# sbelharbi/feature-vs-text-compound-emotion

Hardware: AMD Instinct MI355X
Metric: training clips/sec (32-frame tri-modal clip) (higher is better)
Workload: dtype bf16x3 (split hi/lo bf16 operands, 3 MFMAs per product, fp32 accumulate; <= 2^-15 relative per product)

## Files before the change

feature_vs_text_compound_emotion_amd/csrc/conv_b3.h:

```cpp
#pragma once
#include "conv_common.h"

namespace cer {

typedef __bf16 bf16x8 __attribute__((ext_vector_type(8)));
typedef unsigned int u32x4 __attribute__((ext_vector_type(4)));
typedef __attribute__((address_space(3))) void *lds_ptr_t;

__device__ __forceinline__ bf16x8 as_bf16x8(const u32x4 v) { return __builtin_bit_cast(bf16x8, v); }


typedef float f32x4 __attribute__((ext_vector_type(4)));
__device__ __forceinline__ int swz16(int q) { return (0x78 >> (2 * q)) & 3; }

int conv_b3_patch_launch(int tile, const ConvArgs &a, hipStream_t st);
bool conv_b3_patch_ok(const ConvArgs &a);
bool conv_b3_win_ok(const ConvArgs &a);
int conv_b3_s2d_launch(int tile, const ConvArgs &a, hipStream_t st);
bool conv_b3_s2d_ok(const ConvArgs &a);

}
```

feature_vs_text_compound_emotion_amd/csrc/conv_b3.hip:

```cpp
#include "conv_b3.h"

namespace cer {

template <int BM, int BN, int WP, int WC, int NW = 4, int STAGES = 2>
__global__ __launch_bounds__(NW * 64, NW == 4 ? 2 : 1) void conv_b3_dma16_kernel(ConvArgs p) {
    static_assert(WP * WC == NW && BM % (16 * NW) == 0 && BN % (16 * NW) == 0, "1-KiB pieces are dealt round-robin to the waves");
    constexpr int BKT = 32, ROWB = BKT * 2;
    constexpr int XP = BM / (16 * NW), WQ = BN / (16 * NW);
    constexpr int PX = BM * ROWB, PW = BN * ROWB;
    constexpr int BUF = 2 * PX + 2 * PW;
    constexpr int NDMA = 2 * XP + 2 * WQ;
    static_assert(STAGES == 2 || STAGES == 3, "ring depth");
    constexpr int TP = BM / (16 * WP), TC = BN / (16 * WC);
    constexpr unsigned OOB = 0x80000000u;
    extern __shared__ __attribute__((aligned(16))) uint16_t smem_b3[];
    unsigned char *smem = reinterpret_cast<unsigned char *>(smem_b3);

    const int tid = threadIdx.x, lane = tid & 63;
    const int wave = __builtin_amdgcn_readfirstlane(tid >> 6);
    const int wp = wave % WP, wc = wave / WP;
    const int kg = lane >> 4, l15 = lane & 15;

    const int nwg = p.tiles_m * p.tiles_n;
    int bid = blockIdx.x;
// ... 247 lines not shown
                    const int m = m0 + (wp * TP + b) * 16 + l15;
                    const float v = (m < p.M) ? acc[a][b][r] : 0.f;
                    s1 += v;
                    s2 += v * v;
                });
#pragma unroll
                for (int o = 8; o > 0; o >>= 1) {
                    s1 += __shfl_xor(s1, o);
                    s2 += __shfl_xor(s2, o);
                }
                if (l15 == 0) {
                    const int ci = (wc * TC + a) * 16 + 4 * kg + r;
                    red[(wp * 2 + 0) * BN + ci] = s1;
                    red[(wp * 2 + 1) * BN + ci] = s2;
                }
            });
        });
        __syncthreads();
        if (tid < BN && c0 + tid < p.Cout) {
            float s1 = 0.f, s2 = 0.f;
#pragma unroll
            for (int w = 0; w < WP; ++w) {
                s1 += red[(w * 2 + 0) * BN + tid];
                s2 += red[(w * 2 + 1) * BN + tid];
            }
            p.stats[((size_t)tile_m * 2 + 0) * p.Cout + c0 + tid] = s1;
            p.stats[((size_t)tile_m * 2 + 1) * p.Cout + c0 + tid] = s2;
        }
    }
}

__global__ void split_bf16_kernel(const float4 *__restrict__ x, const float *__restrict__ scale,
                                  const float *__restrict__ shift, ushort4 *__restrict__ hi, ushort4 *__restrict__ lo,
                                  size_t n4, int C4) {
    size_t i = (size_t)blockIdx.x * blockDim.x + threadIdx.x;
    if (i >= n4) return;
    float4 v = x[i];
    if (scale) {
        const int c = (int)(i % C4) * 4;
        const float4 s = *reinterpret_cast<const float4 *>(scale + c), t = *reinterpret_cast<const float4 *>(shift + c);
        v = make_float4(v.x * s.x + t.x, v.y * s.y + t.y, v.z * s.z + t.z, v.w * s.w + t.w);
    }
    ushort4 h, l;
    split_bf16(v.x, h.x, l.x); split_bf16(v.y, h.y, l.y);
    split_bf16(v.z, h.z, l.z); split_bf16(v.w, h.w, l.w);
    hi[i] = h;
    lo[i] = l;
}

template <int BM, int BN, int WP, int WC, int NW = 4, int STAGES = 2>
static int launch_b3_dma16(const ConvArgs &a, hipStream_t st) {
    if ((long long)BN * a.Kpad * 2 >= (1ll << 31))
        return cer_set_error(CER_ERR_UNSUPPORTED, "conv2d (bf16x3, LDS-DMA): weight panel exceeds 31-bit offsets");
    const size_t lds = (size_t)STAGES * (2 * BM + 2 * BN) * 64;
    auto k = conv_b3_dma16_kernel<BM, BN, WP, WC, NW, STAGES>;
    if (lds > 64 * 1024) CER_HIP_CHECK(hipFuncSetAttribute((const void *)k, hipFuncAttributeMaxDynamicSharedMemorySize, (int)lds));
    CER_LAUNCH(k, dim3(a.tiles_m * a.tiles_n, 1, a.split_k), dim3(NW * 64), lds, st, a);
    CER_HIP_CHECK(hipGetLastError());
    return CER_OK;
}

static bool b3_patch_geometry(const cer_conv_desc *d) {
    return d->KH == 3 && d->KW == 3 && d->stride == 1 && d->dil_h == 1 && d->dil_w == 1 && d->pad_t == 1 && d->pad_l == 1 &&
           d->Ho == d->H && d->Wo == d->W && (d->H & 15) == 0 && (d->W & 15) == 0 && (d->Cin & 31) == 0 && d->split_k <= 1;
}

static bool b3_win_geometry(const cer_conv_desc *d) {
    return d->KH == 3 && d->KW == 3 && d->stride == 1 && d->dil_h == 1 && d->dil_w == 1 && d->pad_t == 1 && d->pad_l == 1 &&
           d->Ho == d->H && d->Wo == d->W && d->H >= 2 && d->W >= 2 && d->W <= 86 && (d->Cin & 31) == 0 && d->split_k <= 1;
}

int conv_b3_tile_dims(const cer_conv_desc *d, int &bm, int &bn, int &bk) {
    int tile = d->tile;
    const long long M = (long long)d->N * d->Ho * d->Wo;
    const int Cout = d->Cout;
    if (d->x_s2d) {
        if (tile == 0) tile = Cout > 64 ? 52 : 51;
        else if (tile != 51 && tile != 52) return 0;
    } else if (tile == 51 || tile == 52) {
        return 0;
    }
    if (tile == 0) {
        const long long t128 = (M + 127) / 128 * ((Cout + 127) / 128), t256 = (M + 255) / 256;
        if (b3_patch_geometry(d) && Cout <= 64 && t256 >= 512) tile = 59;
        else if (b3_patch_geometry(d) && Cout >= 128 && t256 * ((Cout + 127) / 128) >= 512) tile = 58;
        else if (b3_win_geometry(d) && t256 >= 64) tile = Cout > 64 ? 56 : 53;
        else if (Cout <= 64) tile = t256 >= 512 ? 48 : 42;
        else if (t128 >= 512) tile = 41;
        else tile = Cout >= 128 ? 44 : 45;
    }
    bk = 32;
    switch (tile) {
        case 41: bm = 128; bn = 128; break;
        case 42: bm = 128; bn = 64; break;
        case 44: bm = 64; bn = 128; break;
        case 45: bm = 64; bn = 64; break;
        case 48: bm = 256; bn = 64; break;
        case 59: bm = 256; bn = 64; break;
        case 58: bm = 256; bn = 128; break;
        case 53: bm = 256; bn = 64; break;
        case 56: bm = 256; bn = 128; break;
        case 51: bm = 256; bn = 64; break;
        case 52: bm = 256; bn = 128; break;
        default: return 0;
    }
    return tile;
}

int conv_b3_launch(int tile, const ConvArgs &a, hipStream_t st) {
    switch (tile) {
        case 41: return launch_b3_dma16<128, 128, 2, 2>(a, st);
        case 42: return launch_b3_dma16<128, 64, 2, 2>(a, st);
        case 44: return launch_b3_dma16<64, 128, 1, 4>(a, st);
        case 45: return launch_b3_dma16<64, 64, 2, 2>(a, st);
        case 48: return launch_b3_dma16<256, 64, 4, 1>(a, st);
        case 53: case 56: case 58: case 59: return conv_b3_patch_launch(tile, a, st);
        case 51: case 52: return conv_b3_s2d_launch(tile, a, st);
        default: return cer_set_error(CER_ERR_INVALID_ARG, "conv2d (bf16x3): unknown tile id");
    }
}

}

using namespace cer;

extern "C" int cer_conv2d_b3_tile(const cer_conv_desc *d) {
    if (!d || d->N <= 0 || d->Ho <= 0 || d->Wo <= 0 || d->Cout <= 0) return 0;
    int bm, bn, bk;
    return conv_b3_tile_dims(d, bm, bn, bk);
}

extern "C" int cer_split_bf16(const float *x, const float *scale, const float *shift, int C, uint16_t *hi, uint16_t *lo,
                              size_t n, void *stream) {
    if (!x || !hi || !lo || n == 0 || (n & 3)) return cer_set_error(CER_ERR_INVALID_ARG, "split_bf16: n must be a positive multiple of 4");
    if ((scale == nullptr) != (shift == nullptr) || (scale && (C <= 0 || (C & 3) || n % C)))
        return cer_set_error(CER_ERR_INVALID_ARG, "split_bf16: the per-channel affine needs scale, shift and C % 4 == 0 dividing n");
    CER_LAUNCH(split_bf16_kernel, dim3(cer_blocks(n / 4, 256)), dim3(256), 0, (hipStream_t)stream, (const float4 *)x, scale,
               shift, (ushort4 *)hi, (ushort4 *)lo, n / 4, scale ? C / 4 : 1);
    CER_HIP_CHECK(hipGetLastError());
    return CER_OK;
}
```

feature_vs_text_compound_emotion_amd/csrc/conv_igemm.hip:

```cpp
#include <hip/hip_runtime.h>
#include <stdint.h>

#include "cer_internal.h"
#include "conv_common.h"

namespace cer {

template <int BM, int BN, int WP, int WC, bool VEC, int VAR, int BKT>
__global__ __launch_bounds__(WP * WC * 64, 3) void conv_igemm_kernel(ConvArgs p) {
    constexpr int NT = WP * WC * 64;
    constexpr int CH = BKT / 4;
    constexpr int RPP = NT / CH;
    constexpr int PIT = BKT + 4;
    constexpr int NG = BKT / 8;
    constexpr bool PRIO = (VAR & 1) != 0, SINGLE = (VAR & 2) != 0, BLKPRIO = (VAR & 4) != 0;
    constexpr bool ABL_NOSTAGE = (VAR & 8) != 0;
    constexpr bool ABL_NOBAR = (VAR & 16) != 0;
    constexpr int NBUF = SINGLE ? 1 : 2;
    constexpr int TP = BM / (32 * WP);
    constexpr int TC = BN / (32 * WC);
    constexpr int XR = BM / RPP;
    constexpr int WR = BN / RPP;
    extern __shared__ __attribute__((aligned(16))) float smem[];
    float *Xs = smem;
// ... 316 lines not shown
        if (t.bn > 64 && d->Cout <= 64) continue;
        const long long blocks = (long long)((M + t.bm - 1) / t.bm) * ((d->Cout + t.bn - 1) / t.bn) * d->split_k;
        const long long slots = 256ll * t.per_cu;
        const long long rounds = (blocks + slots - 1) / slots;
        const float frac = (float)(blocks - (rounds - 1) * slots) / (float)slots;
        const float eff_rounds = (float)(rounds - 1) + (frac < 0.5f ? 0.5f + frac * 0.5f : (frac < 1.f ? 0.75f + frac * 0.25f : 1.f));
        const float time = eff_rounds * (float)(t.bm * t.bn) * (float)t.per_cu / t.rate;
        if (time < best_t) { best_t = time; best = t.id; }
    }
    return best;
}

static void tile_dims(int tile, int &bm, int &bn) {
    switch (tile) {
        case 1: bm = 128; bn = 128; break;
        case 2: bm = 128; bn = 64; break;
        case 4: bm = 64; bn = 128; break;
        default: bm = 64; bn = 64; break;
    }
}

template <int VAR>
static int launch_shape(int shape, const ConvArgs &a, bool vec, hipStream_t st) {
    switch (shape) {
        case 1: return launch_cfg<128, 128, 2, 2, VAR>(a, vec, st);
        case 2: return launch_cfg<128, 64, 2, 2, VAR>(a, vec, st);
        case 4: return launch_cfg<64, 128, 1, 4, VAR>(a, vec, st);
        case 5: return launch_cfg<64, 64, 2, 2, VAR>(a, vec, st);
        default: return cer_set_error(CER_ERR_INVALID_ARG, "conv2d_fwd: unknown tile id");
    }
}

}

using namespace cer;

extern "C" int cer_conv_kpad(int KH, int KW, int Cin) {
    int K = KH * KW * Cin;
    return (K + BK - 1) / BK * BK;
}

static int validate_desc(const cer_conv_desc *d) {
    if (!d) return cer_set_error(CER_ERR_INVALID_ARG, "conv desc is NULL");
    if (d->N <= 0 || d->H <= 0 || d->W <= 0 || d->Cin <= 0 || d->Ho <= 0 || d->Wo <= 0 || d->Cout <= 0 ||
        d->KH <= 0 || d->KW <= 0 || d->stride <= 0 || d->dil_h <= 0 || d->dil_w <= 0 || d->split_k < 1)
        return cer_set_error(CER_ERR_INVALID_ARG, "conv desc: non-positive dimension");
    if ((long long)d->N * d->Ho * d->Wo >= (1ll << 31) || (long long)d->N * d->H * d->W >= (1ll << 31))
        return cer_set_error(CER_ERR_UNSUPPORTED, "conv desc: more than 2^31 pixels");
    if (d->x_nchw && (d->Cin % 32) == 0)
        return cer_set_error(CER_ERR_UNSUPPORTED, "conv desc: NCHW input only on the small-Cin path");
    return CER_OK;
}

namespace cer {
int conv_b3_tile_dims(const cer_conv_desc *d, int &bm, int &bn, int &bk);
int conv_n16_tile_dims(const cer_conv_desc *d, int &bm, int &bn, int &bk);
}

extern "C" int cer_conv2d_stats_tiles(const cer_conv_desc *d, int kernel_family) {
    if (!d || d->N <= 0 || d->Ho <= 0 || d->Wo <= 0) return 0;
    const int M = d->N * d->Ho * d->Wo;
    int bm, bn, bk;
    if (kernel_family == 2) {
        if (!conv_n16_tile_dims(d, bm, bn, bk)) return 0;
    } else if (kernel_family == 1) {
        const int t = conv_b3_tile_dims(d, bm, bn, bk);
        if (!t) return 0;
        if (t == 6) return 2 * ((M + bm - 1) / bm);
    } else {
        tile_dims(pick_tile(d, M), bm, bn);
    }
    return (M + bm - 1) / bm;
}

extern "C" size_t cer_conv2d_workspace_bytes(const cer_conv_desc *d) {
    if (!d || d->split_k <= 1) return 0;
    return (size_t)d->split_k * d->N * d->Ho * d->Wo * d->Cout * sizeof(float);
}

namespace cer {
int conv_b3_launch(int tile, const ConvArgs &a, hipStream_t st);
int conv_n16_launch(int tile, const ConvArgs &a, hipStream_t st);
bool conv_n16_p64_ok(const ConvArgs &a);
}

extern "C" int cer_conv2d_run(const cer_conv_desc *d, const cer_conv_io *io, void *workspace, size_t workspace_bytes,
                              void *stream) {
    int rc = validate_desc(d);
    if (rc) return rc;
    if (!io) return cer_set_error(CER_ERR_INVALID_ARG, "conv2d: io block is NULL");
    if (d->storage != CER_STORE_NONE && d->storage != CER_STORE_BF16 && d->storage != CER_STORE_F16)
        return cer_set_error(CER_ERR_INVALID_ARG, "conv2d: unknown storage type");
    const bool narrow = d->storage != CER_STORE_NONE;
    const bool n16 = narrow && io->x_hi != nullptr;
    const bool b3 = !narrow && io->x_hi != nullptr;
    if (narrow && (io->x_lo || io->w_lo || io->y_lo || io->res_lo || io->y2_hi || io->y2_lo))
        return cer_set_error(CER_ERR_INVALID_ARG, "conv2d (narrow): 16-bit tensors are single planes (every *_lo and y2 pointer must be NULL)");
    if (n16) {
        if (!io->w_hi) return cer_set_error(CER_ERR_INVALID_ARG, "conv2d (narrow): x_hi and w_hi must both be given");
        if (io->in_scale || io->mask || io->aux || d->x_nchw)
            return cer_set_error(CER_ERR_UNSUPPORTED, "conv2d (narrow): no input affine / mask / aux / NCHW input");
    } else if (b3) {
        if (!io->x_lo || !io->w_hi || !io->w_lo)
            return cer_set_error(CER_ERR_INVALID_ARG, "conv2d (bf16x3): x_hi, x_lo, w_hi, w_lo must all be given");
        if (io->in_scale || io->mask || io->aux || d->x_nchw)
            return cer_set_error(CER_ERR_UNSUPPORTED, "conv2d (bf16x3): no input affine / mask / aux / NCHW input");
    } else if (!io->x || !io->w) {
        return cer_set_error(CER_ERR_INVALID_ARG, "conv2d: x and w must be non-NULL");
    }
    if (!io->y && !io->y_hi && !io->y2_hi) return cer_set_error(CER_ERR_INVALID_ARG, "conv2d: no output tensor");
    if ((io->in_scale == nullptr) != (io->in_shift == nullptr))
        return cer_set_error(CER_ERR_INVALID_ARG, "conv2d: in_scale and in_shift go together");
    if (!narrow && ((io->y_hi == nullptr) != (io->y_lo == nullptr) || (io->res_hi == nullptr) != (io->res_lo == nullptr) ||
                    (io->y2_hi == nullptr) != (io->y2_lo == nullptr) || (io->y2_hi && (!io->s2 || !io->t2))))
        return cer_set_error(CER_ERR_INVALID_ARG, "conv2d: split tensors need both planes (and s2/t2 for the second output)");
    if (io->residual && io->res_hi) return cer_set_error(CER_ERR_INVALID_ARG, "conv2d: give the residual as fp32 OR split");
    if (d->act1 == CER_ACT_PRELU && !io->alpha) return cer_set_error(CER_ERR_INVALID_ARG, "conv2d: PReLU needs alpha");
    const bool has_res = io->residual || io->res_hi;
    if (has_res && (d->res_stride <= 0 || d->Hr <= 0 || d->Wr <= 0 || (d->Ho - 1) * d->res_stride >= d->Hr ||
                    (d->Wo - 1) * d->res_stride >= d->Wr))
        return cer_set_error(CER_ERR_INVALID_ARG, "conv2d: residual geometry out of range");
    if (io->stats && d->split_k > 1)
        return cer_set_error(CER_ERR_UNSUPPORTED, "conv2d: batch statistics are not available with split-K");
    if ((io->y_hi || io->y2_hi || io->res_hi) && (d->Cout & 3))
        return cer_set_error(CER_ERR_UNSUPPORTED, "conv2d: split outputs / residual need Cout % 4 == 0");
    ConvArgs a{};
    a.x = io->x; a.w = io->w; a.in_scale = io->in_scale; a.in_shift = io->in_shift; a.bias = io->bias; a.alpha = io->alpha;
    a.res = io->residual; a.mask = io->mask; a.y = io->y; a.aux = io->aux; a.stats = io->stats;
    a.x_hi = io->x_hi; a.x_lo = io->x_lo; a.w_hi = io->w_hi; a.w_lo = io->w_lo;
    a.res_hi = io->res_hi; a.res_lo = io->res_lo; a.y_hi = io->y_hi; a.y_lo = io->y_lo;
    a.s2 = io->s2; a.t2 = io->t2; a.y2_hi = io->y2_hi; a.y2_lo = io->y2_lo;
    a.bias9 = io->bias9;
    a.narrow = d->storage;
    if (io->bias9 && (io->bias || d->stride != 1 || d->Ho != d->H || d->Wo != d->W || d->H < 2 || d->W < 2 || d->split_k > 1))
        return cer_set_error(CER_ERR_INVALID_ARG, "conv2d: bias9 replaces bias and needs a stride-1 same conv on >= 2x2 images without split-K");
    if (d->x_s2d || d->y_s2d) {
        if (!b3 && !n16) return cer_set_error(CER_ERR_UNSUPPORTED, "conv2d: space-to-depth tensors exist in the bf16x3 and narrow modes only");
        if (d->x_s2d && d->x_ld > 0) return cer_set_error(CER_ERR_INVALID_ARG, "conv2d: x_s2d fixes the input pitch (x_ld must be 0)");
        if (d->y_s2d && ((d->Ho | d->Wo) & 1 || io->y || io->y2_hi || has_res || io->mask || io->aux || d->y_ld > 0 || !io->y_hi))
            return cer_set_error(CER_ERR_INVALID_ARG, "conv2d: y_s2d needs even Ho / Wo and a plain 16-bit output (no fp32 / second "
                                                      "output, residual, mask, aux or y_ld)");
    }
    a.x_s2d = d->x_s2d != 0; a.y_s2d = d->y_s2d != 0;
    a.x_ld = d->x_s2d ? 4 * d->Cin : (d->x_ld > 0 ? d->x_ld : d->Cin);
    a.y_ld = d->y_ld > 0 ? d->y_ld : d->Cout;
    if (a.x_ld < d->Cin || a.y_ld < d->Cout || ((d->Cin % 32) == 0 && (a.x_ld & 3) != 0))
        return cer_set_error(CER_ERR_INVALID_ARG, "conv2d: x_ld/y_ld smaller than the channel count or x_ld % 4 != 0");
    if (d->x_nchw && d->x_ld > 0) return cer_set_error(CER_ERR_INVALID_ARG, "conv2d: x_ld is meaningless for NCHW input");
    a.N = d->N; a.H = d->H; a.W = d->W; a.Cin = d->Cin; a.Ho = d->Ho; a.Wo = d->Wo; a.Cout = d->Cout;
    a.KH = d->KH; a.KW = d->KW; a.stride = d->stride; a.dil_h = d->dil_h; a.dil_w = d->dil_w;
    a.pad_t = d->pad_t; a.pad_l = d->pad_l; a.x_nchw = d->x_nchw;
    a.res_stride = d->res_stride; a.Hr = d->Hr; a.Wr = d->Wr; a.act1 = d->act1; a.act2 = d->act2;
    a.slope = d->slope;
    a.Kpad = cer_conv_kpad(d->KH, d->KW, d->Cin);
    a.M = d->N * d->Ho * d->Wo;
    const bool vec = (d->Cin % 32) == 0;
    int tile, bm, bn, bk, esz;
    if (n16) {
        tile = conv_n16_tile_dims(d, bm, bn, bk);
        if (!tile) return cer_set_error(CER_ERR_INVALID_ARG, "conv2d (narrow): unknown tile id (space-to-depth input: 81 / 82 only)");
        if (d->y_s2d && tile != 71 && tile != 72 && tile != 78 && tile != 73 && tile != 76 && tile != 77 && tile != 79)
            return cer_set_error(CER_ERR_UNSUPPORTED, "conv2d (narrow): y_s2d is written by the window / patch kernels only "
                                                      "(cer_conv2d_n16_tile(desc) in {71, 72, 73, 76, 77, 78, 79})");
        if (d->Cin % bk != 0 || (a.x_ld & 7))
            return cer_set_error(CER_ERR_UNSUPPORTED, "conv2d (narrow): Cin must be a multiple of 64 and x_ld of 8");
        esz = 2;
    } else if (b3) {
        tile = conv_b3_tile_dims(d, bm, bn, bk);
        if (!tile) return cer_set_error(CER_ERR_INVALID_ARG, "conv2d (bf16x3): unknown tile id (space-to-depth input: 51 / 52 only)");
        if (d->y_s2d && tile != 53 && tile != 56 && tile != 58 && tile != 59)
            return cer_set_error(CER_ERR_UNSUPPORTED, "conv2d (bf16x3): y_s2d is written by the window / patch kernels only "
                                                      "(cer_conv2d_b3_tile(desc) in {53, 56, 58, 59})");
        if (d->Cin % bk != 0 || (a.x_ld & 7))
            return cer_set_error(CER_ERR_UNSUPPORTED, "conv2d (bf16x3): Cin must be a multiple of the K step and x_ld of 8");
        esz = 2;
    } else {
        tile = pick_tile(d, a.M);
        if (tile != 1 && tile != 2 && tile != 4 && tile != 5) return cer_set_error(CER_ERR_INVALID_ARG, "conv2d: unknown tile id");
        bk = 32;
        tile_dims(tile, bm, bn);
        esz = 4;
    }
    a.cin_steps = (vec || b3 || n16) ? d->Cin / bk : 1;
    a.steps = a.Kpad / bk;
    a.split_k = d->split_k > a.steps ? a.steps : d->split_k;
    a.steps_per_split = (a.steps + a.split_k - 1) / a.split_k;
    a.split_k = (a.steps + a.steps_per_split - 1) / a.steps_per_split;
    a.tiles_m = (a.M + bm - 1) / bm;
    a.tiles_n = (a.Cout + bn - 1) / bn;
    if (vec || b3 || n16) {
        if (d->KH * d->KW > 32) return cer_set_error(CER_ERR_UNSUPPORTED, "conv2d: more than 32 filter taps");
        if (d->Wo > d->W / d->stride + 1 ||
            (long long)d->H * d->W < (long long)(d->Ho - 1) * d->stride * d->W + (long long)(d->Wo - 1) * d->stride)
            return cer_set_error(CER_ERR_UNSUPPORTED, "conv2d: the output grid outruns the input (Ho/Wo too large for H/W and stride)");
        const long long span_px = (long long)bm * d->stride * d->stride + 2ll * d->H * d->W + (long long)d->W * d->stride + 2;
        if (span_px * a.x_ld * esz >= (1ll << 31) || (long long)bn * a.Kpad * esz >= (1ll << 32))
            return cer_set_error(CER_ERR_UNSUPPORTED, "conv2d: tile footprint exceeds 32-bit staging offsets");
    }
    hipStream_t st = (hipStream_t)stream;
    ConvArgs fin = a;
    if (a.split_k > 1) {
        size_t need = (size_t)a.split_k * a.M * a.Cout * sizeof(float);
        if (!workspace || workspace_bytes < need) return cer_set_error(CER_ERR_WORKSPACE, "conv2d: split-K workspace too small");
        a.y = (float *)workspace;
    }
    if (n16) {
        if (tile == 79 && d->tile == 0 && !conv_n16_p64_ok(a)) tile = 71;
        rc = conv_n16_launch(tile, a, st);
    } else if (b3) {
        rc = conv_b3_launch(tile, a, st);
    } else {
        rc = launch_shape<2>(tile, a, vec, st);
    }
    if (rc) return rc;
    if (a.split_k > 1) {
        fin.split_k = a.split_k;
        size_t n = (size_t)a.M * ((a.Cout + 3) / 4);
        CER_LAUNCH(splitk_reduce_kernel, dim3((unsigned)((n + 255) / 256)), dim3(256), 0, st, fin, (const float *)workspace);
        CER_HIP_CHECK(hipGetLastError());
    }
    return CER_OK;
}

extern "C" int cer_conv2d_fwd(const cer_conv_desc *d, const float *x, const float *w, const float *in_scale,
                              const float *in_shift, const float *bias, const float *alpha, const float *residual,
                              const float *mask, float *y, float *aux, float *stats, void *workspace,
                              size_t workspace_bytes, void *stream) {
    if (!x || !w || !y) return cer_set_error(CER_ERR_INVALID_ARG, "conv2d_fwd: x, w, y must be non-NULL");
    cer_conv_io io{};
    io.x = x; io.w = w; io.in_scale = in_scale; io.in_shift = in_shift; io.bias = bias; io.alpha = alpha;
    io.residual = residual; io.mask = mask; io.y = y; io.aux = aux; io.stats = stats;
    return cer_conv2d_run(d, &io, workspace, workspace_bytes, stream);
}
```

feature_vs_text_compound_emotion_amd/ops.py:

```python
import ctypes
import os

import torch

from . import _lib
from ._lib import (ACT_GELU, ACT_LEAKY, ACT_NONE, ACT_PRELU, ACT_RELU, STORE_BF16, STORE_F16, STORE_NONE, ConvDesc,
                   ConvIO, check, current_stream, ptr)

LEAKY_SLOPE = 0.01


def _dev_f32(t, name, contiguous=True, shape=None):
    if t is None:
        return
    if not (t.is_cuda and t.dtype == torch.float32 and (t.is_contiguous() or not contiguous)):
        raise ValueError(f"{name}: expected a contiguous float32 tensor on the GPU, got "
                         f"{t.dtype} {t.device} contiguous={t.is_contiguous()}")
    if shape is not None and tuple(t.shape) != tuple(shape):
        raise ValueError(f"{name}: expected shape {tuple(shape)}, got {tuple(t.shape)}")


def _dev_mask(mask, y):
    _dev_f32(mask, "mask")
    if mask is not None and mask.numel() != y.numel():
# ... 79 lines not shown
            raise ValueError("y_ld needs an explicit out buffer")
        out = _empty((n, ho, wo, cout), x)
    elif out is not None:
        _dev_f32(out, "out", contiguous=(y_ld == 0))
    ws_bytes = lib.cer_conv2d_workspace_bytes(ctypes.byref(d))
    ws = _empty((ws_bytes // 4,), x) if ws_bytes else None
    stats = _empty((lib.cer_conv2d_stats_tiles(ctypes.byref(d), 0), 2, cout), x) if want_stats else None
    if out_n16 is not None:
        if out_split or next_affine is not None:
            raise ValueError("out_n16 excludes the split outputs")
        io = ConvIO()
        io.x, io.w = x.data_ptr(), w_packed.data_ptr()
        for name, t in (("in_scale", in_scale), ("in_shift", in_shift), ("bias", bias), ("alpha", alpha),
                        ("residual", residual), ("mask", mask), ("y", out), ("aux", aux), ("stats", stats)):
            if t is not None:
                setattr(io, name, t.data_ptr())
        d.storage = storage_of(out_n16)
        res = {"y": out, "stats": stats, "n16": torch.empty((n, ho, wo, cout), device=x.device, dtype=out_n16)}
        io.y_hi = res["n16"].data_ptr()
        check(lib.cer_conv2d_run(ctypes.byref(d), ctypes.byref(io), ptr(ws), ws_bytes, current_stream()), "cer_conv2d_run")
        return res
    if not (out_split or next_affine is not None):
        check(lib.cer_conv2d_fwd(ctypes.byref(d), ptr(x), ptr(w_packed), ptr(in_scale), ptr(in_shift), ptr(bias),
                                 ptr(alpha), ptr(residual), ptr(mask), ptr(out), ptr(aux), ptr(stats), ptr(ws), ws_bytes,
                                 current_stream()), "cer_conv2d_fwd")
        return (out, stats) if want_stats else out
    io = ConvIO()
    io.x, io.w = x.data_ptr(), w_packed.data_ptr()
    for name, t in (("in_scale", in_scale), ("in_shift", in_shift), ("bias", bias), ("alpha", alpha),
                    ("residual", residual), ("mask", mask), ("y", out), ("aux", aux), ("stats", stats)):
        if t is not None:
            setattr(io, name, t.data_ptr())
    res = {"y": out, "stats": stats}
    if out_split:
        res["split"] = Split.empty((n, ho, wo, cout), x.device)
        io.y_hi, io.y_lo = res["split"].hi.data_ptr(), res["split"].lo.data_ptr()
    if next_affine is not None:
        s2, t2 = next_affine
        res["next"] = Split.empty((n, ho, wo, cout), x.device)
        io.s2, io.t2 = s2.data_ptr(), t2.data_ptr()
        io.y2_hi, io.y2_lo = res["next"].hi.data_ptr(), res["next"].lo.data_ptr()
    check(lib.cer_conv2d_run(ctypes.byref(d), ctypes.byref(io), ptr(ws), ws_bytes, current_stream()), "cer_conv2d_run")
    return res


class Split:
    __slots__ = ("hi", "lo")

    def __init__(self, hi, lo):
        self.hi, self.lo = hi, lo

    @property
    def shape(self):
        return self.hi.shape

    def float(self):
        return self.hi.float() + self.lo.float()

    def view(self, *shape):
        return Split(self.hi.view(*shape), self.lo.view(*shape))

    @staticmethod
    def empty(shape, device):
        return Split(torch.empty(shape, device=device, dtype=torch.bfloat16),
                     torch.empty(shape, device=device, dtype=torch.bfloat16))


def split_bf16(x, scale=None, shift=None):
    _dev_f32(x, "x")
    _dev_f32(scale, "scale", shape=x.shape[-1:])
    _dev_f32(shift, "shift", shape=x.shape[-1:])
    out = Split.empty(x.shape, x.device)
    c = x.shape[-1] if scale is not None else 0
    check(_lib.load().cer_split_bf16(ptr(x), ptr(scale), ptr(shift), c, ptr(out.hi), ptr(out.lo), x.numel(),
                                     current_stream()), "cer_split_bf16")
    return out


def _dev_bf16(t, name):
    if t is not None and not (t.is_cuda and t.dtype == torch.bfloat16 and t.is_contiguous()):
        raise ValueError(f"{name}: expected a contiguous bfloat16 GPU tensor")


CONV_TRACE = None


def conv2d_b3(x, w, kh, kw, *, stride=1, dil=(1, 1), pad=(0, 0), out_hw=None, bias=None, alpha=None, residual=None,
              res_stride=1, act1=ACT_NONE, act2=ACT_NONE, slope=LEAKY_SLOPE, split_k=1, tile=0, out_f32=False,
              out_split=True, next_affine=None, want_stats=False, bias9=None, x_s2d=False, y_s2d=False):
    lib = _lib.load()
    for t, n in ((x.hi, "x.hi"), (x.lo, "x.lo"), (w.hi, "w.hi"), (w.lo, "w.lo")):
        _dev_bf16(t, n)
    _dev_f32(bias, "bias")
    _dev_f32(alpha, "alpha")
    n, h, wd, cin = x.shape
    if x_s2d:
        if cin % 4:
            raise ValueError("a space-to-depth input has 4 * Cin channels")
        h, wd, cin = 2 * h, 2 * wd, cin // 4
    cout = w.shape[0]
    if w.shape[1] != conv_kpad(kh, kw, cin):
        raise ValueError(f"packed weight has K={w.shape[1]}, expected {conv_kpad(kh, kw, cin)}")
    if out_hw is None:
        ho = (h + 2 * pad[0] - dil[0] * (kh - 1) - 1) // stride + 1
        wo = (wd + 2 * pad[1] - dil[1] * (kw - 1) - 1) // stride + 1
    else:
        ho, wo = out_hw
    d = ConvDesc()
    d.N, d.H, d.W, d.Cin, d.Ho, d.Wo, d.Cout = n, h, wd, cin, ho, wo, cout
    d.KH, d.KW, d.stride, d.dil_h, d.dil_w, d.pad_t, d.pad_l = kh, kw, stride, dil[0], dil[1], pad[0], pad[1]
    d.res_stride, d.Hr, d.Wr = res_stride, 0, 0
    d.act1, d.act2, d.slope, d.split_k, d.tile = act1, act2, slope, split_k, tile
    d.x_s2d, d.y_s2d = int(x_s2d), int(y_s2d)
    io = ConvIO()
    io.x_hi, io.x_lo, io.w_hi, io.w_lo = x.hi.data_ptr(), x.lo.data_ptr(), w.hi.data_ptr(), w.lo.data_ptr()
    io.bias = bias.data_ptr() if bias is not None else None
    io.alpha = alpha.data_ptr() if alpha is not None else None
    if bias9 is not None:
        _dev_f32(bias9, "bias9")
        if tuple(bias9.shape) != (9, cout):
            raise ValueError("bias9 must be [9, Cout]")
        io.bias9 = bias9.data_ptr()
    if residual is not None:
        rshape = residual.shape
        if rshape[0] != n or rshape[3] != cout:
            raise ValueError("residual shape does not match the output")
        d.Hr, d.Wr = rshape[1], rshape[2]
        if isinstance(residual, Split):
            _dev_bf16(residual.hi, "residual.hi")
            io.res_hi, io.res_lo = residual.hi.data_ptr(), residual.lo.data_ptr()
        else:
            _dev_f32(residual, "residual")
            io.residual = residual.data_ptr()
    res = {}
    dev = x.hi.device
    if out_f32:
        res["y"] = torch.empty((n, ho, wo, cout), device=dev, dtype=torch.float32)
        io.y = res["y"].data_ptr()
    if out_split:
        res["split"] = Split.empty((n, ho // 2, wo // 2, 4 * cout) if y_s2d else (n, ho, wo, cout), dev)
        io.y_hi, io.y_lo = res["split"].hi.data_ptr(), res["split"].lo.data_ptr()
    if next_affine is not None:
        s2, t2 = next_affine
        _dev_f32(s2, "s2")
        _dev_f32(t2, "t2")
        res["next"] = Split.empty((n, ho, wo, cout), dev)
        io.s2, io.t2 = s2.data_ptr(), t2.data_ptr()
        io.y2_hi, io.y2_lo = res["next"].hi.data_ptr(), res["next"].lo.data_ptr()
    if want_stats:
        res["stats"] = torch.empty((lib.cer_conv2d_stats_tiles(ctypes.byref(d), 1), 2, cout), device=dev,
                                   dtype=torch.float32)
        io.stats = res["stats"].data_ptr()
    ws_bytes = lib.cer_conv2d_workspace_bytes(ctypes.byref(d))
    ws = torch.empty((ws_bytes // 4,), device=dev, dtype=torch.float32) if ws_bytes else None
    if CONV_TRACE is not None:
        e0, e1 = torch.cuda.Event(enable_timing=True), torch.cuda.Event(enable_timing=True)
        e0.record()
    check(lib.cer_conv2d_run(ctypes.byref(d), ctypes.byref(io), ptr(ws), ws_bytes, current_stream()), "cer_conv2d_run")
    if CONV_TRACE is not None:
        e1.record()
        nout = n * ho * wo * cout
        nbytes = 4.0 * n * h * wd * cin + 4.0 * nout * (int(out_f32) + int(out_split) + int(next_affine is not None)) + \
            4.0 * cout * cin * kh * kw + (4.0 * nout if residual is not None else 0.0)
        CONV_TRACE.append((lib.cer_conv2d_b3_tile(ctypes.byref(d)), 2.0 * n * ho * wo * cout * cin * kh * kw, e0, e1, nbytes))
    return res


def stem_conv(x, w, scale=None, shift=None, alpha=None, out=None, want_stats=False):
    _dev_f32(x, "x")
    _dev_f32(w, "w")
    for t, nme in ((scale, "scale"), (shift, "shift"), (alpha, "alpha")):
        _dev_f32(t, nme)
    n, c, h, wd = x.shape
    if c != 3 or w.shape[0] != 64:
        raise ValueError("stem_conv is the 3 -> 64 input layer")
    lib = _lib.load()
    stats = _empty((lib.cer_stem_conv3x3_stats_rows(n, h), 2, 64), x) if (want_stats or out is None) else None
    res, y, hi, lo, storage = {}, None, None, None, STORE_NONE
    if out == "f32":
        res["y"] = y = torch.empty((n, h, wd, 64), device=x.device, dtype=torch.float32)
    elif out == "split":
        res["split"] = Split.empty((n, h, wd, 64), x.device)
        hi, lo = res["split"].hi, res["split"].lo
    elif out is not None:
        storage = storage_of(out)
        res["n16"] = hi = torch.empty((n, h, wd, 64), device=x.device, dtype=out)
    check(lib.cer_stem_conv3x3(ptr(x), ptr(w), w.shape[1], ptr(scale), ptr(shift), ptr(alpha), ptr(y), ptr(hi), ptr(lo), storage,
                               ptr(stats), n, h, wd, current_stream()), "cer_stem_conv3x3")
    if out is None:
        return stats
    if want_stats:
        res["stats"] = stats
    return res


def _tile_desc(n, h, w, cin, cout, kh, kw, stride, pad, x_s2d):
    d = ConvDesc()
    d.N, d.H, d.W, d.Cin, d.Cout = n, h, w, cin, cout
    d.Ho, d.Wo = (h + 2 * pad[0] - kh) // stride + 1, (w + 2 * pad[1] - kw) // stride + 1
    d.KH, d.KW, d.stride, d.dil_h, d.dil_w, d.pad_t, d.pad_l = kh, kw, stride, 1, 1, pad[0], pad[1]
    d.split_k, d.x_s2d = 1, int(x_s2d)
    return d


def conv2d_b3_tile(n, h, w, cin, cout, kh, kw, stride, pad, x_s2d=False):
    return _lib.load().cer_conv2d_b3_tile(ctypes.byref(_tile_desc(n, h, w, cin, cout, kh, kw, stride, pad, x_s2d)))


def conv2d_n16_tile(n, h, w, cin, cout, kh, kw, stride, pad, x_s2d=False):
    return _lib.load().cer_conv2d_n16_tile(ctypes.byref(_tile_desc(n, h, w, cin, cout, kh, kw, stride, pad, x_s2d)))


S2D_PRODUCER_TILES = (53, 56, 58, 59)
S2D_PRODUCER_TILES_N16 = (71, 72, 73, 76, 77, 78, 79)


def s2d_k_order(cin, device, chunk=32):
    order = (ctypes.c_int32 * (9 * cin))()
    check(_lib.load().cer_conv_s2d_k_order(cin, chunk, order), "cer_conv_s2d_k_order")
    return torch.tensor(list(order), dtype=torch.long, device=device)


def pack_s2d_weight(w, cin, chunk=None):
    if isinstance(w, Split):
        idx = s2d_k_order(cin, w.hi.device, chunk or 32)
        return Split(w.hi.index_select(1, idx).contiguous(), w.lo.index_select(1, idx).contiguous())
    return w.index_select(1, s2d_k_order(cin, w.device, chunk or 64)).contiguous()


def space_to_depth(x):
    if isinstance(x, Split):
        return Split(space_to_depth(x.hi), space_to_depth(x.lo))
    return torch.cat([x[:, 1::2, 1::2], x[:, 1::2, 0::2], x[:, 0::2, 1::2], x[:, 0::2, 0::2]], dim=3).contiguous()


def storage_of(dtype):
    if dtype == torch.bfloat16:
        return STORE_BF16
    if dtype == torch.float16:
        return STORE_F16
    raise ValueError(f"narrow storage is torch.bfloat16 or torch.float16, got {dtype}")


def _dev_n16(t, name, dtype=None):
    if t is None:
        return
    if not (t.is_cuda and t.dtype in (torch.bfloat16, torch.float16) and t.is_contiguous()) or (dtype is not None and t.dtype != dtype):
        raise ValueError(f"{name}: expected a contiguous {dtype or 'bfloat16/float16'} GPU tensor, got {t.dtype} {t.device}")


def to_n16(x, dtype, scale=None, shift=None):
    _dev_f32(x, "x")
    _dev_f32(scale, "scale", shape=x.shape[-1:])
    _dev_f32(shift, "shift", shape=x.shape[-1:])
    out = torch.empty(x.shape, device=x.device, dtype=dtype)
    c = x.shape[-1] if scale is not None else 0
    check(_lib.load().cer_to_n16(ptr(x), ptr(scale), ptr(shift), c, ptr(out), x.numel(), storage_of(dtype), current_stream()),
          "cer_to_n16")
    return out


def from_n16(x):
    _dev_n16(x, "x")
    out = torch.empty(x.shape, device=x.device, dtype=torch.float32)
    check(_lib.load().cer_from_n16(ptr(x), ptr(out), x.numel(), storage_of(x.dtype), current_stream()), "cer_from_n16")
    return out


def conv2d_n16(x, w, kh, kw, *, stride=1, dil=(1, 1), pad=(0, 0), out_hw=None, bias=None, alpha=None, residual=None,
               res_stride=1, act1=ACT_NONE, act2=ACT_NONE, slope=LEAKY_SLOPE, split_k=1, tile=0, out_f32=False,
               out_n16=True, want_stats=False, bias9=None, x_s2d=False, y_s2d=False):
    lib = _lib.load()
    _dev_n16(x, "x")
    _dev_n16(w, "w", x.dtype)
    _dev_f32(bias, "bias")
    _dev_f32(alpha, "alpha")
    n, h, wd, cin = x.shape
    if x_s2d:
        if cin % 4:
            raise ValueError("a space-to-depth input has 4 * Cin channels")
        h, wd, cin = 2 * h, 2 * wd, cin // 4
    cout = w.shape[0]
    if w.shape[1] != conv_kpad(kh, kw, cin):
        raise ValueError(f"packed weight has K={w.shape[1]}, expected {conv_kpad(kh, kw, cin)}")
    if out_hw is None:
        ho = (h + 2 * pad[0] - dil[0] * (kh - 1) - 1) // stride + 1
        wo = (wd + 2 * pad[1] - dil[1] * (kw - 1) - 1) // stride + 1
    else:
        ho, wo = out_hw
    d = ConvDesc()
    d.N, d.H, d.W, d.Cin, d.Ho, d.Wo, d.Cout = n, h, wd, cin, ho, wo, cout
    d.KH, d.KW, d.stride, d.dil_h, d.dil_w, d.pad_t, d.pad_l = kh, kw, stride, dil[0], dil[1], pad[0], pad[1]
    d.res_stride, d.Hr, d.Wr = res_stride, 0, 0
    d.act1, d.act2, d.slope, d.split_k, d.tile = act1, act2, slope, split_k, tile
    d.storage = storage_of(x.dtype)
    d.x_s2d, d.y_s2d = int(x_s2d), int(y_s2d)
# ... 989 lines not shown
```

Baseline: 57.95.

## Add persistent two-group patch kernel for bf16x3 Cin=64, Cout=64 3x3 convs

Adds a persistent 512-thread kernel for bf16x3 3x3 stride-1 convolutions with Cin=64 and Cout=64 on large images. It keeps all nine weight taps resident in LDS and splits the workgroup into two wave groups that alternate between MFMA compute phases and halo-window DMA/epilogue phases on 16x16 patches. The grid is sized to the CU count and patches are spread across XCDs. The goal is to hide global loads and stores behind compute and to avoid reloading weights per tile. The cost is a large, barrier-heavy schedule and a narrow eligibility check, with a fallback to tiles 58/59 when the check fails.

```diff
diff --git a/feature_vs_text_compound_emotion_amd/csrc/conv_b3.h b/feature_vs_text_compound_emotion_amd/csrc/conv_b3.h
--- a/feature_vs_text_compound_emotion_amd/csrc/conv_b3.h
+++ b/feature_vs_text_compound_emotion_amd/csrc/conv_b3.h
@@ -16,6 +16,8 @@
 int conv_b3_patch_launch(int tile, const ConvArgs &a, hipStream_t st);
 bool conv_b3_patch_ok(const ConvArgs &a);
 bool conv_b3_win_ok(const ConvArgs &a);
+int conv_b3_p64_launch(const ConvArgs &a, hipStream_t st);
+bool conv_b3_p64_ok(const ConvArgs &a);
 int conv_b3_s2d_launch(int tile, const ConvArgs &a, hipStream_t st);
 bool conv_b3_s2d_ok(const ConvArgs &a);
 
diff --git a/feature_vs_text_compound_emotion_amd/csrc/conv_b3.hip b/feature_vs_text_compound_emotion_amd/csrc/conv_b3.hip
--- a/feature_vs_text_compound_emotion_amd/csrc/conv_b3.hip
+++ b/feature_vs_text_compound_emotion_amd/csrc/conv_b3.hip
@@ -353,7 +353,8 @@
     }
     if (tile == 0) {
         const long long t128 = (M + 127) / 128 * ((Cout + 127) / 128), t256 = (M + 255) / 256;
-        if (b3_patch_geometry(d) && Cout <= 64 && t256 >= 512) tile = 59;
+        if (b3_patch_geometry(d) && d->Cin == 64 && Cout == 64 && t256 >= 2048) tile = 57;
+        else if (b3_patch_geometry(d) && Cout <= 64 && t256 >= 512) tile = 59;
         else if (b3_patch_geometry(d) && Cout >= 128 && t256 * ((Cout + 127) / 128) >= 512) tile = 58;
         else if (b3_win_geometry(d) && t256 >= 64) tile = Cout > 64 ? 56 : 53;
         else if (Cout <= 64) tile = t256 >= 512 ? 48 : 42;
@@ -367,6 +368,7 @@
         case 44: bm = 64; bn = 128; break;
         case 45: bm = 64; bn = 64; break;
         case 48: bm = 256; bn = 64; break;
+        case 57: bm = 256; bn = 64; break;
         case 59: bm = 256; bn = 64; break;
         case 58: bm = 256; bn = 128; break;
         case 53: bm = 256; bn = 64; break;
@@ -386,6 +388,7 @@
         case 45: return launch_b3_dma16<64, 64, 2, 2>(a, st);
         case 48: return launch_b3_dma16<256, 64, 4, 1>(a, st);
         case 53: case 56: case 58: case 59: return conv_b3_patch_launch(tile, a, st);
+        case 57: return conv_b3_p64_launch(a, st);
         case 51: case 52: return conv_b3_s2d_launch(tile, a, st);
         default: return cer_set_error(CER_ERR_INVALID_ARG, "conv2d (bf16x3): unknown tile id");
     }
diff --git a/feature_vs_text_compound_emotion_amd/csrc/conv_b3_p64.hip b/feature_vs_text_compound_emotion_amd/csrc/conv_b3_p64.hip
--- /dev/null
+++ b/feature_vs_text_compound_emotion_amd/csrc/conv_b3_p64.hip
@@ -0,0 +1,336 @@
+#include "conv_b3.h"
+
+namespace cer {
+
+namespace {
+constexpr int BP_BN = 64, BP_XPP = 21, BP_XPL = BP_XPP * 1024, BP_XBYTES = 2 * BP_XPL;
+constexpr int BP_WPL = BP_BN * 64, BP_WSLICE = 2 * BP_WPL;
+constexpr int BP_WOFF = 2 * BP_XBYTES, BP_SINK = BP_WOFF + 9 * BP_WSLICE;
+constexpr int BP_LDS = BP_SINK + 1024;
+constexpr unsigned long long BP_F_TABLE = 0xaaa00a00ull;
+__device__ __forceinline__ int bp_f(int wx) { return (int)((BP_F_TABLE >> (2 * wx)) & 3ull); }
+struct BpGeo { FastDiv tiles_n, pxn, pyn; };
+}
+
+__global__ __launch_bounds__(512, 2) void conv_b3_p64_kernel(ConvArgs p, BpGeo geo) {
+    constexpr int BN = BP_BN, NWG = 4, WP = 4, TP = 4, TC = 4, PH = 16, PWD = 16, WW = 18, WROWS = 18 * 18;
+    constexpr int XPP = BP_XPP, XPW = (XPP + NWG - 1) / NWG, XPL = BP_XPL, XBYTES = BP_XBYTES;
+    constexpr int NWIN = 2 * XPW;
+    constexpr int WPL = BP_WPL, WSLICE = BP_WSLICE, WOFF = BP_WOFF, SINK = BP_SINK;
+    constexpr unsigned OOB = 0x80000000u;
+    extern __shared__ __attribute__((aligned(16))) uint16_t smem_bp64[];
+    unsigned char *smem = reinterpret_cast<unsigned char *>(smem_bp64);
+
+    const int tid = threadIdx.x, lane = tid & 63;
+    const int wave = __builtin_amdgcn_readfirstlane(tid >> 6);
+    const int grp = wave >> 2, wp = wave & 3;
+    const int kg = lane >> 4, l15 = lane & 15;
+    const int prow = lane >> 2, slot = lane & 3;
+
+    const int xcd = blockIdx.x & 7, kblk = blockIdx.x >> 3, nbx = gridDim.x >> 3;
+    const int kq = (int)fdiv((unsigned)kblk, geo.tiles_n), tile_n = kblk - kq * p.tiles_n;
+    const int pstride = nbx / p.tiles_n;
+    const int q8 = p.tiles_m >> 3, r8 = p.tiles_m & 7;
+    const int plo = xcd * q8 + (xcd < r8 ? xcd : r8), pcnt = q8 + (xcd < r8 ? 1 : 0);
+    const int c0 = tile_n * BN;
+    if (kq >= pcnt) return;
+    const int nblk = (pcnt - kq + pstride - 1) / pstride;
+    const int nmine = (nblk - grp + 1) >> 1;
+
+    const size_t wpan = (size_t)c0 * p.Kpad * 2;
+    const char *wh = reinterpret_cast<const char *>(p.w_hi) + wpan, *wl = reinterpret_cast<const char *>(p.w_lo) + wpan;
+    unsigned w_off;
+    {
+        const int row = wp * 16 + prow;
+        w_off = (unsigned)(epi_cout_of_row(row) * p.Kpad * 2) + (unsigned)((slot ^ swz16((row >> 2) & 3)) << 4);
+    }
+    auto issue_w3 = [&](int cc, int tap0) __attribute__((always_inline)) {
+#pragma unroll
+        for (int i = 0; i < 3; ++i) {
+            const size_t koff = ((size_t)(tap0 + i) * p.Cin + (size_t)cc * 32) * 2;
+            const __amdgpu_buffer_rsrc_t rh = __builtin_amdgcn_make_buffer_rsrc(const_cast<char *>(wh) + koff, 0, (int)OOB, 0x00020000);
+            const __amdgpu_buffer_rsrc_t rl = __builtin_amdgcn_make_buffer_rsrc(const_cast<char *>(wl) + koff, 0, (int)OOB, 0x00020000);
+            unsigned char *dst = smem + WOFF + (tap0 + i) * WSLICE + wp * 1024;
+            __builtin_amdgcn_raw_ptr_buffer_load_lds(rh, (lds_ptr_t)dst, 16, (int)w_off, 0, 0, 0);
+            __builtin_amdgcn_raw_ptr_buffer_load_lds(rl, (lds_ptr_t)(dst + WPL), 16, (int)w_off, 0, 0, 0);
+        }
+    };
+
+    const int pitch = p.x_ld * 2;
+    int wyx[XPW];
+    unsigned xrel[XPW];
+#pragma unroll
+    for (int i = 0; i < XPW; ++i) {
+        const int qp = wp + NWG * i;
+        const int row = qp * 16 + prow;
+        const int wy = row / WW, wx = row - wy * WW;
+        const bool live = qp < XPP && row < WROWS;
+        wyx[i] = live ? wy * 32 + wx : -1;
+        xrel[i] = live ? (unsigned)((wy * p.W + wx) * pitch) + (unsigned)((slot ^ bp_f(wx)) << 4) : OOB;
+    }
+    struct Patch { int n, py, px, id; };
+    auto patch_of = [&](int jj) __attribute__((always_inline)) {
+        Patch t;
+        t.id = plo + kq + (2 * jj + grp) * pstride;
+        const int prw = (int)fdiv((unsigned)t.id, geo.pxn);
+        t.px = t.id - prw * (int)geo.pxn.d;
+        t.n = (int)fdiv((unsigned)prw, geo.pyn);
+        t.py = prw - t.n * (int)geo.pyn.d;
+        return t;
+    };
+    auto issue_window = [&](const Patch &t, int cc) __attribute__((always_inline)) {
+        const int iy0 = t.py * PH - 1, ix0 = t.px * PWD - 1;
+        const int base = (iy0 * p.W + ix0) * pitch;
+        const bool interior = t.py > 0 && t.py < (int)geo.pyn.d - 1 && t.px > 0 && t.px < (int)geo.pxn.d - 1;
+        const size_t img = (size_t)t.n * p.H * p.W * p.x_ld * 2 + (size_t)cc * 64;
+        const __amdgpu_buffer_rsrc_t rh = __builtin_amdgcn_make_buffer_rsrc(
+            const_cast<char *>(reinterpret_cast<const char *>(p.x_hi) + img), 0, (int)OOB, 0x00020000);
+        const __amdgpu_buffer_rsrc_t rl = __builtin_amdgcn_make_buffer_rsrc(
+            const_cast<char *>(reinterpret_cast<const char *>(p.x_lo) + img), 0, (int)OOB, 0x00020000);
+#pragma unroll
+        for (int i = 0; i < XPW; ++i) {
+            bool inb = wyx[i] >= 0;
+            if (!interior) {
+                const int iy = iy0 + (wyx[i] >> 5), ix = ix0 + (wyx[i] & 31);
+                inb = inb && (unsigned)iy < (unsigned)p.H && (unsigned)ix < (unsigned)p.W;
+            }
+            const bool real = wp + NWG * i < XPP;
+            const int vo = (int)(real && inb ? (unsigned)(base + (int)xrel[i]) : OOB);
+            unsigned char *dst = real ? smem + grp * XBYTES + (wp + NWG * i) * 1024 : smem + SINK;
+            __builtin_amdgcn_raw_ptr_buffer_load_lds(rh, (lds_ptr_t)dst, 16, vo, 0, 0, 0);
+            __builtin_amdgcn_raw_ptr_buffer_load_lds(rl, (lds_ptr_t)(real ? dst + XPL : dst), 16, vo, 0, 0, 0);
+        }
+    };
+
+    const int arow = WOFF + l15 * 64 + ((kg ^ swz16((l15 >> 2) & 3)) << 4);
+    int bcol[3];
+#pragma unroll
+    for (int kw = 0; kw < 3; ++kw) bcol[kw] = (wp * WW + kw + l15) * 64 + ((kg ^ bp_f(kw + l15)) << 4);
+    const unsigned char *Xb = smem + grp * XBYTES;
+    const int emode = epi_mode(p);
+
+    f32x4 acc[TC][TP];
+    float s1[2][8], s2[2][8];
+
+    auto phase_barrier = [&]() __attribute__((always_inline)) {
+        __builtin_amdgcn_sched_barrier(0);
+        __builtin_amdgcn_s_barrier();
+        __builtin_amdgcn_sched_barrier(0);
+    };
+
+    auto k_phase = [&](bool live) __attribute__((always_inline)) {
+        u32x4 af[2][2][TC], bf[2][2][TP];
+        auto read_tap = [&](auto T, int set) {
+            constexpr int tap = decltype(T)::v, kh = tap / 3, kw = tap % 3;
+#pragma unroll
+            for (int a = 0; a < TC; ++a) {
+                af[set][0][a] = *reinterpret_cast<const u32x4 *>(smem + tap * WSLICE + arow + a * 16 * 64);
+                af[set][1][a] = *reinterpret_cast<const u32x4 *>(smem + tap * WSLICE + WPL + arow + a * 16 * 64);
+            }
+#pragma unroll
+            for (int b = 0; b < TP; ++b) {
+                bf[set][0][b] = *reinterpret_cast<const u32x4 *>(Xb + kh * (WW * 64) + bcol[kw] + b * WP * WW * 64);
+                bf[set][1][b] = *reinterpret_cast<const u32x4 *>(Xb + XPL + kh * (WW * 64) + bcol[kw] + b * WP * WW * 64);
+            }
+        };
+        if (!live) {
+            phase_barrier();
+            phase_barrier();
+            phase_barrier();
+            return;
+        }
+        read_tap(IdxC<0>{}, 0);
+        __builtin_amdgcn_sched_group_barrier(0x100, 16, 0);
+        static_for<9>([&](auto T) {
+            constexpr int tap = decltype(T)::v, set = tap & 1;
+            if constexpr (tap < 8) read_tap(IdxC<tap + 1>{}, set ^ 1);
+#pragma unroll
+            for (int g = 0; g < TP; ++g)
+#pragma unroll
+                for (int a = 0; a < TC; ++a) {
+                    acc[a][g] = __builtin_amdgcn_mfma_f32_16x16x32_bf16(as_bf16x8(af[set][1][a]), as_bf16x8(bf[set][0][g]), acc[a][g], 0, 0, 0);
+                    acc[a][g] = __builtin_amdgcn_mfma_f32_16x16x32_bf16(as_bf16x8(af[set][0][a]), as_bf16x8(bf[set][1][g]), acc[a][g], 0, 0, 0);
+                    acc[a][g] = __builtin_amdgcn_mfma_f32_16x16x32_bf16(as_bf16x8(af[set][0][a]), as_bf16x8(bf[set][0][g]), acc[a][g], 0, 0, 0);
+                }
+            if constexpr (tap < 8) {
+#pragma unroll
+                for (int g = 0; g < 4; ++g) {
+                    __builtin_amdgcn_sched_group_barrier(0x100, 4, 0);
+                    __builtin_amdgcn_sched_group_barrier(0x008, 12, 0);
+                }
+            }
+            if constexpr (tap % 3 == 2) {
+                asm volatile("s_waitcnt lgkmcnt(0)" ::: "memory");
+                phase_barrier();
+            }
+        });
+    };
+
+    auto walk = [&](auto MODE_, auto STATS_) __attribute__((always_inline)) {
+        constexpr int MODE = decltype(MODE_)::v;
+        constexpr bool STATS = decltype(STATS_)::v;
+        constexpr int NST = 16;
+        float aa[2][8], bb[2][8];
+        epi_direct_consts<MODE>(p, c0 + kg * 8, aa[0], bb[0]);
+        epi_direct_consts<MODE>(p, c0 + 32 + kg * 8, aa[1], bb[1]);
+        if constexpr (STATS) {
+#pragma unroll
+            for (int j = 0; j < 2; ++j)
+#pragma unroll
+                for (int e = 0; e < 8; ++e) s1[j][e] = s2[j][e] = 0.f;
+        }
+        const int last_id = plo + kq + (nblk - 1) * pstride;
+        auto stores = [&](const Patch &t) __attribute__((always_inline)) {
+            if constexpr (STATS) {
+                if (t.id != last_id && (tid & 255) < 2 * BN)
+                    p.stats[((size_t)t.id * 2 + ((tid & 255) >> 6)) * p.Cout + c0 + (tid & 63)] = 0.f;
+            }
+            static_for<8>([&](auto CH) {
+                constexpr int ch = decltype(CH)::v, b = ch / 2, j = ch % 2;
+                const int c = c0 + j * 32 + kg * 8;
+                const int gy = t.py * PH + b * WP + wp, gx = t.px * PWD + l15;
+                const int m = (t.n * p.H + gy) * p.W + gx;
+                int cs = 4;
+                if constexpr (MODE == EPI_B9_PRELU_SPLIT) {
+                    const int ry = gy == 0 ? 0 : (gy == p.H - 1 ? 2 : 1), rx = gx == 0 ? 0 : (gx == p.W - 1 ? 2 : 1);
+                    cs = 3 * ry + rx;
+                }
+                const float v[8] = {acc[2 * j][b][0], acc[2 * j][b][1], acc[2 * j][b][2], acc[2 * j][b][3],
+                                    acc[2 * j + 1][b][0], acc[2 * j + 1][b][1], acc[2 * j + 1][b][2], acc[2 * j + 1][b][3]};
+                if constexpr (STATS) {
+#pragma unroll
+                    for (int e = 0; e < 8; ++e) {
+                        s1[j][e] += v[e];
+                        s2[j][e] += v[e] * v[e];
+                    }
+                }
+                const size_t orow = (size_t)(p.y_s2d ? s2d_row(m, gy, gx, p.W) : m);
+                if constexpr (MODE == EPI_B9_PRELU_SPLIT) {
+                    if (__ballot(cs != 4) != 0ull) epi_direct8<MODE, CER_STORE_BF16, true>(p, aa[j], bb[j], orow, c, cs, v);
+                    else epi_direct8<MODE, CER_STORE_BF16, false>(p, aa[j], bb[j], orow, c, 4, v);
+                } else {
+                    epi_direct8<MODE, CER_STORE_BF16, false>(p, aa[j], bb[j], orow, c, cs, v);
+                }
+            });
+        };
+
+        Patch cur = patch_of(0), nxt = cur;
+        if (nmine > 0) issue_window(cur, 0);
+        if (grp == 0) { issue_w3(0, 0); issue_w3(0, 3); } else { issue_w3(0, 6); }
+        asm volatile("s_waitcnt vmcnt(0)" ::: "memory");
+        phase_barrier();
+        const int nph = 4 * ((nblk + 1) >> 1) + 1;
+        for (int ph = 0; ph < nph; ++ph) {
+            const int t = ph - grp, role = t & 3, jj = t >> 2;
+            const bool live = jj >= 0 && jj < nmine;
+            if ((role & 1) == 0) {
+                if (role == 0) {
+#pragma unroll
+                    for (int a = 0; a < TC; ++a)
+#pragma unroll
+                        for (int b = 0; b < TP; ++b) acc[a][b] = f32x4{0.f, 0.f, 0.f, 0.f};
+                }
+                k_phase(live);
+            } else {
+                const int wcc = role == 1 ? 1 : 0;
+                bool win = false;
+                if (role == 1) {
+                    win = live;
+                } else if (live) {
+                    win = jj + 1 < nmine;
+                    if (win) nxt = patch_of(jj + 1);
+                }
+                const bool st = role == 3 && live;
+                if (grp == 0) {
+                    if (win) issue_window(role == 1 ? cur : nxt, wcc);
+                    phase_barrier();
+                    issue_w3(wcc, 0);
+                    phase_barrier();
+                    issue_w3(wcc, 3);
+                } else {
+                    issue_w3(wcc, 6);
+                    __builtin_amdgcn_sched_barrier(0);
+                    if (win) issue_window(role == 1 ? cur : nxt, wcc);
+                    __builtin_amdgcn_sched_barrier(0);
+                    if (win) asm volatile("s_waitcnt vmcnt(%0)" ::"n"(NWIN) : "memory");
+                    else asm volatile("s_waitcnt vmcnt(0)" ::: "memory");
+                    phase_barrier();
+                    phase_barrier();
+                }
+                __builtin_amdgcn_sched_barrier(0);
+                if (st) {
+                    stores(cur);
+                    __builtin_amdgcn_sched_barrier(0);
+                    asm volatile("s_waitcnt vmcnt(%0)" ::"n"(NST) : "memory");
+                    cur = nxt;
+                } else {
+                    asm volatile("s_waitcnt vmcnt(0)" ::: "memory");
+                }
+                phase_barrier();
+            }
+        }
+        if constexpr (STATS) {
+#pragma unroll
+            for (int j = 0; j < 2; ++j)
+#pragma unroll
+                for (int e = 0; e < 8; ++e) {
+                    s1[j][e] = row16_sum(s1[j][e]);
+                    s2[j][e] = row16_sum(s2[j][e]);
+                }
+            float *red = reinterpret_cast<float *>(smem);
+            if (l15 == 0) {
+#pragma unroll
+                for (int j = 0; j < 2; ++j) {
+                    float *d1 = red + (wave * 2 + 0) * BN + j * 32 + kg * 8, *d2 = d1 + BN;
+                    *reinterpret_cast<float4 *>(d1) = make_float4(s1[j][0], s1[j][1], s1[j][2], s1[j][3]);
+                    *reinterpret_cast<float4 *>(d1 + 4) = make_float4(s1[j][4], s1[j][5], s1[j][6], s1[j][7]);
+                    *reinterpret_cast<float4 *>(d2) = make_float4(s2[j][0], s2[j][1], s2[j][2], s2[j][3]);
+                    *reinterpret_cast<float4 *>(d2 + 4) = make_float4(s2[j][4], s2[j][5], s2[j][6], s2[j][7]);
+                }
+            }
+            __syncthreads();
+            if (tid < 2 * BN) {
+                const int st = tid >> 6, c = tid & 63;
+                float a = 0.f;
+#pragma unroll
+                for (int w = 0; w < 8; ++w) a += red[(w * 2 + st) * BN + c];
+                p.stats[((size_t)last_id * 2 + st) * p.Cout + c0 + c] = a;
+            }
+        }
+    };
+    if (emode == EPI_RAW_F32) {
+        if (p.stats) walk(IdxC<EPI_RAW_F32>{}, IdxC<1>{});
+        else walk(IdxC<EPI_RAW_F32>{}, IdxC<0>{});
+    } else if (emode == EPI_B9_PRELU_SPLIT) {
+        walk(IdxC<EPI_B9_PRELU_SPLIT>{}, IdxC<0>{});
+    }
+}
+
+bool conv_b3_p64_ok(const ConvArgs &a) {
+    if (!conv_b3_patch_ok(a) || a.Cin != 64 || (a.Cout & 63) || a.tiles_n > 4 || (a.tiles_n & (a.tiles_n - 1)) ||
+        a.tiles_n * BP_BN != a.Cout)
+        return false;
+    const int mode = epi_mode(a);
+    return mode == EPI_RAW_F32 || (mode == EPI_B9_PRELU_SPLIT && !a.stats);
+}
+
+int conv_b3_p64_launch(const ConvArgs &a, hipStream_t st) {
+    if (!conv_b3_p64_ok(a))
+        return cer_set_error(CER_ERR_UNSUPPORTED, "conv2d (bf16x3, persistent patch kernel): needs a 3x3 / stride 1 / pad 1 conv on images whose "
+                                                   "height and width are multiples of 16, Cin == 64, Cout in {64, 128, 256} and the raw fp32 "
+                                                   "or the bias9 + PReLU -> split epilogue");
+    int dev = 0, cus = 0;
+    CER_HIP_CHECK(hipGetDevice(&dev));
+    CER_HIP_CHECK(hipDeviceGetAttribute(&cus, hipDeviceAttributeMultiprocessorCount, dev));
+    const int unit = 8 * a.tiles_n;
+    const int grid = cus / unit * unit;
+    if (grid <= 0) return cer_set_error(CER_ERR_UNSUPPORTED, "conv2d (bf16x3, persistent patch kernel): fewer CUs than 8 x cout tiles");
+    const BpGeo geo{make_fastdiv((unsigned)a.tiles_n), make_fastdiv((unsigned)(a.W / 16)), make_fastdiv((unsigned)(a.H / 16))};
+    auto k = conv_b3_p64_kernel;
+    CER_HIP_CHECK(hipFuncSetAttribute((const void *)k, hipFuncAttributeMaxDynamicSharedMemorySize, BP_LDS));
+    CER_LAUNCH(k, dim3(grid), dim3(512), BP_LDS, st, a, geo);
+    CER_HIP_CHECK(hipGetLastError());
+    return CER_OK;
+}
+
+}
diff --git a/feature_vs_text_compound_emotion_amd/csrc/conv_igemm.hip b/feature_vs_text_compound_emotion_amd/csrc/conv_igemm.hip
--- a/feature_vs_text_compound_emotion_amd/csrc/conv_igemm.hip
+++ b/feature_vs_text_compound_emotion_amd/csrc/conv_igemm.hip
@@ -422,6 +422,7 @@
 int conv_b3_launch(int tile, const ConvArgs &a, hipStream_t st);
 int conv_n16_launch(int tile, const ConvArgs &a, hipStream_t st);
 bool conv_n16_p64_ok(const ConvArgs &a);
+bool conv_b3_p64_ok(const ConvArgs &a);
 }
 
 extern "C" int cer_conv2d_run(const cer_conv_desc *d, const cer_conv_io *io, void *workspace, size_t workspace_bytes,
@@ -508,9 +509,9 @@
     } else if (b3) {
         tile = conv_b3_tile_dims(d, bm, bn, bk);
         if (!tile) return cer_set_error(CER_ERR_INVALID_ARG, "conv2d (bf16x3): unknown tile id (space-to-depth input: 51 / 52 only)");
-        if (d->y_s2d && tile != 53 && tile != 56 && tile != 58 && tile != 59)
+        if (d->y_s2d && tile != 53 && tile != 56 && tile != 57 && tile != 58 && tile != 59)
             return cer_set_error(CER_ERR_UNSUPPORTED, "conv2d (bf16x3): y_s2d is written by the window / patch kernels only "
-                                                      "(cer_conv2d_b3_tile(desc) in {53, 56, 58, 59})");
+                                                      "(cer_conv2d_b3_tile(desc) in {53, 56, 57, 58, 59})");
         if (d->Cin % bk != 0 || (a.x_ld & 7))
             return cer_set_error(CER_ERR_UNSUPPORTED, "conv2d (bf16x3): Cin must be a multiple of the K step and x_ld of 8");
         esz = 2;
@@ -548,6 +549,10 @@
         if (tile == 79 && d->tile == 0 && !conv_n16_p64_ok(a)) tile = 71;
         rc = conv_n16_launch(tile, a, st);
     } else if (b3) {
+        if (tile == 57 && d->tile == 0 && !conv_b3_p64_ok(a)) {
+            tile = a.Cout > 64 ? 58 : 59;
+            a.tiles_n = (a.Cout + (tile == 58 ? 128 : 64) - 1) / (tile == 58 ? 128 : 64);
+        }
         rc = conv_b3_launch(tile, a, st);
     } else {
         rc = launch_shape<2>(tile, a, vec, st);
diff --git a/feature_vs_text_compound_emotion_amd/ops.py b/feature_vs_text_compound_emotion_amd/ops.py
--- a/feature_vs_text_compound_emotion_amd/ops.py
+++ b/feature_vs_text_compound_emotion_amd/ops.py
@@ -185,6 +185,8 @@
         raise ValueError(f"{name}: expected a contiguous bfloat16 GPU tensor")
 
 
+B3_PERSISTENT_PATCH = True
+
 CONV_TRACE = None
 
 
@@ -215,6 +217,8 @@
     d.res_stride, d.Hr, d.Wr = res_stride, 0, 0
     d.act1, d.act2, d.slope, d.split_k, d.tile = act1, act2, slope, split_k, tile
     d.x_s2d, d.y_s2d = int(x_s2d), int(y_s2d)
+    if tile == 0 and not B3_PERSISTENT_PATCH and lib.cer_conv2d_b3_tile(ctypes.byref(d)) == 57:
+        d.tile = 58 if cout > 64 else 59
     io = ConvIO()
     io.x_hi, io.x_lo, io.w_hi, io.w_lo = x.hi.data_ptr(), x.lo.data_ptr(), w.hi.data_ptr(), w.lo.data_ptr()
     io.bias = bias.data_ptr() if bias is not None else None
@@ -314,7 +318,7 @@
     return _lib.load().cer_conv2d_n16_tile(ctypes.byref(_tile_desc(n, h, w, cin, cout, kh, kw, stride, pad, x_s2d)))
 
 
-S2D_PRODUCER_TILES = (53, 56, 58, 59)
+S2D_PRODUCER_TILES = (53, 56, 57, 58, 59)
 S2D_PRODUCER_TILES_N16 = (71, 72, 73, 76, 77, 78, 79)
 
 
```

After: 58.78 (median of 6 runs). 1.01x the previous value.
